# hzxie/GaussianCity

Measured on AMD Instinct MI355X. Metric: rendered frames/sec (fwd) @ 5000000 Gaussians, 1920x1080, higher is better.
Workload: dtype f32; 1 GPU; C3: s_city 5000000 Gaussians, 1920x1080, SH degree 3, forward, 24-pose orbit; exp=gcr-fp32-v2 (bit-exact vs oracle), tile_sort=lists beyond 1024 entries sorted lazily, as far as the blend walks (default), cull=stateless: every frame reads means, scales, rotations (default)

## Files before the change

### gaussiancity_amd/_native.py

```python
import ctypes as C
import subprocess

from . import _loader

GRAD_REC_FLOATS = 16

STAGE_NAMES = ("preprocess", "scan", "emit", "sort", "ranges", "blend_fwd", "blend_bwd",
               "preprocess_bwd")


class Options(C.Structure):
    _fields_ = [(n, C.c_int32) for n in (
        "lazy_sort", "sort_in_blend", "bwd_piece", "deterministic_backward", "split_preprocess",
        "force_radix", "force_global_cursor", "bwd_wave_units")]

    def __init__(self, **kw):
        super().__init__(*([-1] * 8))
        for k, v in kw.items():
            if k not in dict(self._fields_):
                raise TypeError("unknown rasterizer option %r" % k)
            setattr(self, k, int(v))


class Camera(C.Structure):
# ... 25 lines not shown
    ]


class Grads(C.Structure):
    _fields_ = [(n, C.c_void_p) for n in (
        "dL_dmeans2D", "dL_dconic", "dL_dopacity", "dL_dcolors", "dL_dmeans3D", "dL_dcov3D",
        "dL_dsh", "dL_dscales", "dL_drotations")] + [
        ("stride_means3D", C.c_int32), ("stride_opacity", C.c_int32), ("stride_colors", C.c_int32),
        ("stride_scales", C.c_int32), ("stride_rotations", C.c_int32),
        ("packed", C.c_void_p), ("packed_floats", C.c_int64)]


class Layout(C.Structure):
    _fields_ = [
        ("geom_rec", C.c_size_t), ("geom_cov3D", C.c_size_t), ("geom_clamped", C.c_size_t),
        ("geom_tiles_touched", C.c_size_t), ("geom_block_sums", C.c_size_t),
        ("geom_vis_list", C.c_size_t), ("geom_vis_count", C.c_size_t),
        ("geom_num_rendered", C.c_size_t), ("geom_block_tiles", C.c_size_t), ("geom_total", C.c_size_t),
        ("img_final_T", C.c_size_t), ("img_n_contrib", C.c_size_t), ("img_ranges", C.c_size_t),
        ("img_tile_cursor", C.c_size_t), ("img_tile_table", C.c_size_t), ("img_tile_lazy", C.c_size_t),
        ("img_total", C.c_size_t),
        ("bin_keys", C.c_size_t * 2), ("bin_vals", C.c_size_t * 2), ("bin_hist", C.c_size_t),
        ("bin_sorted", C.c_size_t), ("bin_work", C.c_size_t), ("bin_mask", C.c_size_t), ("bin_ckpt", C.c_size_t),
        ("bin_total", C.c_size_t), ("bin_lean_total", C.c_size_t), ("bin_staged", C.c_size_t),
        ("geom_vis_rec", C.c_size_t),
    ]


class FrameInfo(C.Structure):
    _fields_ = [("num_rendered", C.c_int64), ("max_tile_instances", C.c_int64)]


ABI_VERSION = 9
TICKET_WORDS = 8
RESIZE_FN = C.CFUNCTYPE(C.c_void_p, C.c_void_p, C.c_size_t)

_vp, _sz, _i32, _i64, _u32, _int = C.c_void_p, C.c_size_t, C.c_int32, C.c_int64, C.c_uint32, C.c_int
_cam, _gs, _info, _opts = C.POINTER(Camera), C.POINTER(Gaussians), C.POINTER(FrameInfo), C.POINTER(Options)
_SIGNATURES = {
    "gcr_abi_version": (_int, []),
    "gcr_last_error": (C.c_char_p, []),
    "gcr_geometry_bytes": (_sz, [_i32]),
    "gcr_image_bytes": (_sz, [_i32, _i32]),
    "gcr_binning_bytes": (_sz, [_i64, _i32, _i32]),
    "gcr_binning_bytes_lean": (_sz, [_i64, _i32, _i32]),
    "gcr_get_layout": (_int, [_i32, _i32, _i32, _i64, C.POINTER(Layout)]),
    "gcr_forward": (_int, [_cam, _gs, _vp, _sz, _vp, _sz, _i64, _i64, _vp, _sz, _vp, _vp, _info, _vp]),
    "gcr_forward_preprocess": (_int, [_cam, _gs, _vp, _sz, _vp, _sz, _vp, _info, _vp]),
    "gcr_forward_render": (_int, [_cam, _gs, _vp, _sz, _vp, _sz, _vp, _sz, _info, _vp, _vp]),
    "gcr_backward": (_int, [_cam, _gs, _vp, _vp, _sz, _vp, _sz, _vp, _sz, _i64, _vp, C.POINTER(Grads), _vp]),
    "gcr_build_cull_cache": (_int, [_gs, C.c_float, _vp, _vp]),
    "gcr_cull_cache_bytes": (_sz, [_i32]),
    "gcr_mark_visible": (_int, [_i32, _vp, _vp, _vp, _vp, _vp]),
    "gcr_rasterize_forward": (_i64, [RESIZE_FN, _vp, RESIZE_FN, _vp, RESIZE_FN, _vp, _cam, _gs, _vp, _vp, _vp]),
    "gcr_set_option": (_int, [C.c_char_p, _int]),
    "gcr_get_option": (_int, [C.c_char_p]),
    "gcr_get_stage_ms": (_int, [C.POINTER(C.c_float), _int]),
    "gcr_grad_record_floats": (_int, []),
    "gcr_grad_record_floats_opt": (_int, [_opts]),
    "gcr_forward_async": (_int, [_cam, _gs, _vp, _sz, _vp, _sz, _i64, _i64, _vp, _sz, _vp, _vp, _vp, _u32, _vp]),
    "gcr_ticket_poll": (_int, [_vp, _u32, _i64, _info]),
    "gcr_ticket_wait": (_int, [_vp, _u32, _i64, _vp, _info]),
    "gcr_host_words_alloc": (_vp, [_sz]),
    "gcr_host_words_free": (None, [_vp]),
    "gcr_rescue_count": (C.c_long, []),
    "gcr_rescue_dropped_count": (C.c_long, []),
# ... 34 lines not shown
```

### gaussiancity_amd/csrc/gcr_api.hip

```cpp
#include <atomic>
#include <chrono>
#include <condition_variable>
#include <cstdio>
#include <cstring>
#include <deque>
#include <map>
#include <mutex>
#include <string>
#include <thread>

#include <pthread.h>

#include "gcr_internal.h"
#define GC_ERR_HIP GCR_ERR_DEVICE
#include "gc_host.h"

namespace {

std::atomic<int> g_timing{0};
std::atomic<int> g_force_radix{0};
std::atomic<int> g_force_global_cursor{0};
std::atomic<int> g_lazy_sort{1};
std::atomic<int> g_sort_in_blend{0};
std::atomic<int> g_split_preprocess{0};
// ... 274 lines not shown

template <class A>
void set_gaussian_args(A& a, const gcr_gaussians* g) {
  a.P = g->P;
  a.means3D = g->means3D; a.scales = g->scales; a.rotations = g->rotations;
  a.s_mean = stride_or(g->stride_means3D, 3);
  a.s_scale = stride_or(g->stride_scales, 3);
  a.s_rot = stride_or(g->stride_rotations, 4);
}
template <class A>
void set_camera_args(A& a, const gcr_camera* cam, const gcr_gaussians* g) {
  set_gaussian_args(a, g);
  a.D = cam->sh_degree; a.M = g->M; a.W = cam->img_w; a.H = cam->img_h;
  a.tanfovx = cam->tanfovx; a.tanfovy = cam->tanfovy;
  a.focal_y = cam->img_h / (2.0f * cam->tanfovy);
  a.focal_x = cam->img_w / (2.0f * cam->tanfovx);
  a.scale_modifier = cam->scale_modifier;
  a.shs = g->shs;
  a.view = cam->view_matrix; a.proj = cam->proj_matrix; a.campos = cam->campos;
  fill_cam(a.cam, cam);
}

GcrBlendArgs blend_args(const FrameSetup& f, const gcr_camera* cam, const uint32_t* list) {
  GcrBlendArgs b;
  memset(&b, 0, sizeof(b));
  b.ranges = f.ranges;
  b.list = list;
  b.rec = f.rec;
  b.W = cam->img_w; b.H = cam->img_h; b.gx = f.gx; b.gy = f.gy;
  b.bg = cam->bg;
  b.flip_x = cam->flip_x != 0; b.flip_y = cam->flip_y != 0;
  b.win_x = cam->win_x; b.win_y = cam->win_y; b.win_w = cam->win_w; b.win_h = cam->win_h;
  b.out_u8 = cam->out_u8 != 0 && cam->backward != 1;
  fill_cam(b.cam, cam);
  b.final_T = f.final_T;
  b.n_contrib = f.n_contrib;
  return b;
}

}

extern "C" {

#ifdef GCR_EXPERIMENTS
void gcr_debug_set_clock_buffer(void* dev_ptr) { g_clock_buf.store((unsigned long long*)dev_ptr); }
#endif

int gcr_abi_version(void) { return GCR_ABI_VERSION; }
int gcr_grad_record_floats(void) { return g_deterministic.load() ? GCR_GRAD_REC_FLOATS_DET : GCR_GRAD_REC_FLOATS; }
int gcr_grad_record_floats_opt(const gcr_options* options) {
  return resolve_options(options).deterministic ? GCR_GRAD_REC_FLOATS_DET : GCR_GRAD_REC_FLOATS;
}
const char* gcr_last_error(void) { return g_err.c_str(); }

size_t gcr_geometry_bytes(int32_t P) { return compute_layout(P, 16, 16, 0).geom_total; }
size_t gcr_image_bytes(int32_t W, int32_t H) { return compute_layout(0, W, H, 0).img_total; }
size_t gcr_binning_bytes(int64_t R, int32_t W, int32_t H) { return compute_layout(0, W, H, R).bin_total; }
size_t gcr_binning_bytes_lean(int64_t R, int32_t W, int32_t H) { return compute_layout(0, W, H, R).bin_lean_total; }
int gcr_get_layout(int32_t P, int32_t W, int32_t H, int64_t R, gcr_layout* out) {
  if (!out) return fail(GCR_ERR_INVALID_ARGUMENT, "null layout");
  *out = compute_layout(P, W, H, R);
  return 0;
}

int gcr_set_option(const char* name, int value) {
  const OptionRow* o = find_option(name);
// ... 323 lines not shown
  std::condition_variable idle_cv_;

  static void publish(unsigned long long* w, int idx, unsigned int seq) {
    std::atomic_thread_fence(std::memory_order_seq_cst);
    ((volatile unsigned long long*)w)[idx] = (unsigned long long)seq;
    std::atomic_thread_fence(std::memory_order_seq_cst);
  }

  void rescue(AsyncFrame& f) {
    volatile unsigned long long* w = f.words;
    publish(f.words, 7, f.seq);
    if ((unsigned int)w[4] == f.seq) {
      publish(f.words, 5, f.seq);
      publish(f.words, 2, f.seq);
      dropped_.fetch_add(1);
      return;
    }
    const unsigned long long R = w[0] & 0xffffffffull;
    bool ok = false;
    void* stale = nullptr;
    do {
      if (check_num_rendered(R)) break;
      if (hipSetDevice(f.device) != hipSuccess) break;
      const int d = f.device & 63;
      if (!streams_[d]) {
        int lo = 0, hi = 0;
        if (hipDeviceGetStreamPriorityRange(&lo, &hi) != hipSuccess) lo = hi = 0;
        if (hipStreamCreateWithPriority(&streams_[d], hipStreamNonBlocking, hi) != hipSuccess &&
            hipStreamCreateWithFlags(&streams_[d], hipStreamNonBlocking) != hipSuccess)
          break;
      }
      hipStream_t s = streams_[d];
      gcr_camera cam = f.cam;
      cam.backward = 0;
      cam.options = f.has_opt ? &f.opt : nullptr;
      if (cam.host_camera) {
        cam.view_matrix = f.camvals;
        cam.proj_matrix = f.camvals + 16;
        cam.campos = f.camvals + 32;
        cam.bg = f.camvals + 35;
      }
      const FrameSetup fs = frame_setup(resolve_options(cam.options), f.g.P, &cam, 0, f.geom, f.img, nullptr);
      gcr_frame_info info;
      info.num_rendered = (int64_t)R;
      unsigned long long longest = 0;
      if (hipMemcpyAsync(&longest, fs.frame + 1, 8, hipMemcpyDeviceToHost, s) != hipSuccess) break;
      if (hipStreamSynchronize(s) != hipSuccess) break;
      info.max_tile_instances = (int64_t)longest;
      const size_t bytes = gcr_binning_bytes_lean((int64_t)R, cam.img_w, cam.img_h);
      if (scratch_bytes_[d] < bytes) {
        stale = scratch_[d];
        scratch_[d] = nullptr;
        scratch_bytes_[d] = 0;
        if (hipMalloc(&scratch_[d], bytes + bytes / 2) != hipSuccess) {
          scratch_[d] = nullptr;
          break;
        }
        scratch_bytes_[d] = bytes + bytes / 2;
      }
      if (gcr_forward_render(&cam, &f.g, f.geom, f.geom_bytes, scratch_[d], scratch_bytes_[d], f.img, f.img_bytes, &info,
                             f.out_color, s) < 0)
        break;
      if (hipStreamSynchronize(s) != hipSuccess) break;
      ok = true;
    } while (false);
    if (!ok) publish(f.words, 5, f.seq);
    publish(f.words, 6, f.seq);
// ... 428 lines not shown
```

### gaussiancity_amd/csrc/gcr_binning.hip

```cpp
#include <stdlib.h>
#include "gcr_device.h"
#include "gcr_internal.h"
#include "gcr_sort.h"

namespace {

constexpr int SORT_THREADS = 256;
constexpr int SORT_ITEMS = 16;
constexpr int SORT_TILE = SORT_THREADS * SORT_ITEMS;
constexpr int RADIX_BITS = 8;
constexpr int RADIX = 1 << RADIX_BITS;

__global__ __launch_bounds__(256) void k_emit(int P, const uint32_t* __restrict__ tiles_touched,
                                              const uint32_t* __restrict__ block_offsets,
                                              const float4* __restrict__ rec, int gx,
                                              uint64_t* __restrict__ keys,
                                              uint32_t* __restrict__ vals) {
  __shared__ uint32_t lds4[4];
  const int idx = blockIdx.x * 256 + threadIdx.x;
  const uint32_t t = idx < P ? tiles_touched[idx] : 0u;
  uint32_t total;
  uint32_t off = gcr_block_excl_scan_256(t, lds4, &total);
  if (t == 0) return;
  off += block_offsets[blockIdx.x];
// ... 54 lines not shown
      lo = mid;
    else
      hi = mid;
  }
  return (uint32_t)lo * (uint32_t)chunk + (f - pre[lo]);
}
GCR_DEV uint4 tt_survivor(const uint32_t* pre, int nblocks, const uint4* __restrict__ vis_rec, int chunk, uint32_t f) {
  return vis_rec[tt_position(pre, nblocks, chunk, f)];
}

template <bool SCATTER, int TT_THREADS>
__global__ __launch_bounds__(TT_THREADS) void k_tile_table(int T, int gx, int G, int nblocks_k1, int chunk,
                                                           const uint4* __restrict__ vis_rec,
                                                           const uint32_t* __restrict__ vis_count,
                                                           uint32_t* __restrict__ table,
                                                           const uint32_t* __restrict__ tile_total,
                                                           const uint32_t* __restrict__ tile_local,
                                                           const uint32_t* __restrict__ blk_total,
                                                           uint32_t* __restrict__ ranges,
                                                           uint64_t* __restrict__ pairs,
                                                           unsigned long long* __restrict__ frame,
                                                           unsigned long long cap_instances,
                                                           unsigned long long cap_list,
                                                           unsigned long long* __restrict__ host_word,
                                                           unsigned int seq,
                                                           const unsigned long long* __restrict__ block_tiles,
                                                           const uint4* __restrict__ banded, int banded_capacity) {
  extern __shared__ __attribute__((aligned(16))) unsigned char gcr_smem[];
  uint32_t* cnt = reinterpret_cast<uint32_t*>(gcr_smem);
  __shared__ uint32_t pre[GCR_K1_MAX_BLOCKS + 1];
  __shared__ uint32_t blk_base[TT_MAX_TBLOCKS];
  __shared__ uint32_t wtot[TT_THREADS / 64];
  const int tid = threadIdx.x, lane = tid & 63, w = tid >> 6;
  uint32_t* __restrict__ row = table + (size_t)blockIdx.x * T;
  TtPrefix<TT_THREADS> blocks;
  blocks.load(vis_count, nblocks_k1, tid);
  if (!SCATTER) {
    if (blockIdx.x == 0) {
      unsigned long long part = 0ull, pf = 0ull;
      for (int b = tid; b < nblocks_k1; b += TT_THREADS) {
        const unsigned long long v = block_tiles[b];
        part += v & ~GCR_PREFILTER_FLAG;
        pf |= v & GCR_PREFILTER_FLAG;
      }
#pragma unroll
      for (int o = 32; o > 0; o >>= 1) part += __shfl_xor(part, o, 64);
      __shared__ unsigned long long wpart[TT_THREADS / 64];
      if (lane == 0) wpart[w] = part;
      const int prefilter_violation = __syncthreads_or(pf != 0ull ? 1 : 0);
      if (tid == 0) {
        unsigned long long total = 0ull;
#pragma unroll
        for (int k = 0; k < TT_THREADS / 64; k++) total += wpart[k];
        if (prefilter_violation) total = GCR_PREFILTER_MARK;
        frame[0] = total;
        frame[1] = 0ull;
        frame[2] = 0ull;
        frame[GCR_FRAME_PIECE] = 0ull;
        frame[GCR_FRAME_BANDED] = banded != nullptr ? 1ull : 0ull;
        if (host_word != nullptr)
          gcr_store_to_host(host_word, ((unsigned long long)seq << 32) | (total > 0xffffffffull ? 0xffffffffull : total));
      }
    }
    for (int t = tid; t < T; t += TT_THREADS) cnt[t] = 0u;
  } else {
    const bool go = frame[0] <= cap_instances && frame[1] <= cap_list;
    if (blockIdx.x == 0 && tid == 0) {
// ... 500 lines not shown
  k_emit<<<(P + 255) / 256, 256, 0, s>>>(P, tiles_touched, block_offsets, rec, gx, keys, vals);
  return hipGetLastError();
}

bool gcr_band_sort_possible(int T) { return T >= GCR_BANDS; }

int gcr_tile_table_groups(int T, int nblocks_k1, int* G_out) {
  const size_t lds = (size_t)T * sizeof(uint32_t);
  if (lds > 148 * 1024 || (T + 63) / 64 > TT_MAX_TBLOCKS) return 0;
  int ng = 128;
#ifdef GCR_EXPERIMENTS
  if (const char* e = getenv("GCR_TT_GROUPS")) ng = atoi(e);
#endif
  if (ng > nblocks_k1) ng = nblocks_k1;
  if (ng < 1) ng = 1;
  int G = (nblocks_k1 + ng - 1) / ng;
  *G_out = G;
  return (nblocks_k1 + G - 1) / G;
}

static hipError_t tile_table_attr() {
  static hipError_t done = [] {
    const void* fns[4] = {(const void*)k_tile_table<false, 512>, (const void*)k_tile_table<true, 512>,
                          (const void*)k_tile_table<false, 1024>, (const void*)k_tile_table<true, 1024>};
    for (const void* f : fns) {
      const hipError_t e = hipFuncSetAttribute(f, hipFuncAttributeMaxDynamicSharedMemorySize, 148 * 1024);
      if (e != hipSuccess) return e;
    }
    return hipSuccess;
  }();
  return done;
}
static inline bool tile_table_wide(int) { return true; }

hipError_t gcr_launch_tile_count(int T, int gx, int NG, int G, int nblocks_k1, int chunk, const uint4* vis_rec,
                                 const uint32_t* vis_count, uint32_t* table,
                                 uint32_t* tile_total, uint32_t* tile_local, uint32_t* blk_total,
                                 unsigned long long* frame, const unsigned long long* block_tiles,
                                 unsigned long long* host_R, unsigned int seq, uint4* banded, int banded_capacity,
                                 hipStream_t s) {
  hipError_t e = tile_table_attr();
  if (e != hipSuccess) return e;
  if (banded != nullptr) {
    const uint32_t band_mul = (uint32_t)((((uint64_t)GCR_BANDS << 32) + (uint64_t)T - 1) / (uint64_t)T);
    k_band<false><<<BAND_CUTS, BAND_THREADS, 0, s>>>(gx, band_mul, nblocks_k1, chunk, vis_rec, vis_count, table, nullptr,
                                                      banded_capacity);
    k_band<true><<<BAND_CUTS, BAND_THREADS, 0, s>>>(gx, band_mul, nblocks_k1, chunk, vis_rec, vis_count, table, banded,
                                                     banded_capacity);
  }
  if (tile_table_wide(T))
    k_tile_table<false, 1024><<<NG, 1024, (size_t)T * sizeof(uint32_t), s>>>(
        T, gx, G, nblocks_k1, chunk, vis_rec, vis_count, table, nullptr, nullptr, nullptr, nullptr, nullptr,
        frame, 0ull, 0ull, host_R, seq, block_tiles, banded, banded_capacity);
  else
    k_tile_table<false, 512><<<NG, 512, (size_t)T * sizeof(uint32_t), s>>>(
        T, gx, G, nblocks_k1, chunk, vis_rec, vis_count, table, nullptr, nullptr, nullptr, nullptr, nullptr,
        frame, 0ull, 0ull, host_R, seq, block_tiles, banded, banded_capacity);
  k_table_colscan<<<(T + 63) / 64, 1024, 0, s>>>(table, NG, T, tile_total, tile_local, blk_total, frame);
  return hipGetLastError();
}

hipError_t gcr_launch_tile_scatter(int T, int gx, int NG, int G, int nblocks_k1, int chunk, const uint4* vis_rec,
                                   const uint32_t* vis_count, uint32_t* table,
                                   const uint32_t* tile_total, const uint32_t* tile_local,
                                   const uint32_t* blk_total, uint32_t* ranges, uint64_t* pairs,
                                   unsigned long long* frame, unsigned long long cap_instances,
                                   unsigned long long cap_list, unsigned long long* host_longest,
                                   const uint4* banded, int banded_capacity, hipStream_t s) {
  hipError_t e = tile_table_attr();
  if (e != hipSuccess) return e;
  if (tile_table_wide(T))
    k_tile_table<true, 1024><<<NG, 1024, (size_t)T * sizeof(uint32_t), s>>>(
        T, gx, G, nblocks_k1, chunk, vis_rec, vis_count, table, tile_total, tile_local, blk_total, ranges, pairs,
        frame, cap_instances, cap_list, host_longest, 0u, nullptr, banded, banded_capacity);
  else
    k_tile_table<true, 512><<<NG, 512, (size_t)T * sizeof(uint32_t), s>>>(
        T, gx, G, nblocks_k1, chunk, vis_rec, vis_count, table, tile_total, tile_local, blk_total, ranges, pairs,
        frame, cap_instances, cap_list, host_longest, 0u, nullptr, banded, banded_capacity);
  return hipGetLastError();
}

__global__ __launch_bounds__(256) void k_restore_cursors(const uint32_t* __restrict__ ranges,
                                                         uint32_t* __restrict__ cursor, int T) {
  const int t = blockIdx.x * 256 + threadIdx.x;
  if (t < T) cursor[(size_t)t * GCR_CURSOR_STRIDE] = ranges[2 * t];
}

hipError_t gcr_launch_scatter_instances(int nblocks, int chunk, const uint32_t* vis_list,
                                        const uint32_t* vis_count, const float4* rec, int gx,
                                        uint32_t* tile_cursor, uint64_t* pairs, const uint32_t* ranges, int T,
                                        const unsigned long long* frame, hipStream_t s) {
  if (nblocks <= 0) return hipSuccess;
  if (frame == nullptr)
    k_restore_cursors<<<(T + 255) / 256, 256, 0, s>>>(ranges, tile_cursor, T);
  k_scatter_instances<<<nblocks, 256, 0, s>>>(chunk, vis_list, vis_count, rec, gx, tile_cursor, pairs, frame);
  return hipGetLastError();
}

__global__ __launch_bounds__(256) void k_fill_tiles_touched(int chunk, const uint32_t* __restrict__ vis_list,
                                                            const uint32_t* __restrict__ vis_count,
                                                            const float4* __restrict__ rec,
                                                            uint32_t* __restrict__ tiles_touched) {
  const uint32_t nvis = vis_count[blockIdx.x];
  const uint32_t* __restrict__ my_list = vis_list + (size_t)blockIdx.x * chunk;
  for (uint32_t it = threadIdx.x; it < nvis; it += 256) {
    const uint32_t idx = my_list[it];
    const float4 q2 = rec[(size_t)idx * GCR_REC_QUADS + 2];
    const uint32_t rx = __float_as_uint(q2.z), ry = __float_as_uint(q2.w);
    tiles_touched[idx] = ((rx >> 16) - (rx & 0xffffu)) * ((ry >> 16) - (ry & 0xffffu));
  }
// ... 86 lines not shown
```

### gaussiancity_amd/csrc/gcr_blend.hip

```cpp
#include "gcr_cull.h"
#include "gcr_device.h"
#include "gcr_internal.h"
#include "gcr_sort.h"

namespace {

constexpr int CHUNK = 256;
constexpr uint32_t ENTRY_BYTES = 48;
constexpr int K6_SENT_SLOT = 223;
constexpr int K6_LIST_STRIDE = 232;
static_assert(GCR_PIECE_MAX <= K6_SENT_SLOT, "a K6 chunk must leave slot 255 to the sentinel");
constexpr uint32_t NO_ENTRY = 0xFFFFFFFFu;

struct __attribute__((aligned(16))) StagedEntry {
  float4 a, b, c;
};
static_assert(sizeof(StagedEntry) == ENTRY_BYTES, "StagedEntry must be 48 bytes");

GCR_DEV float gcr_alpha_skip_bound(float opacity) {
  if (!(opacity > 0.0f)) return __builtin_inff();
  return gcr_max(-87.0f, -__builtin_logf(255.0f * opacity) - 1.0e-3f);
}

GCR_DEV float blend_exp(float x) { return gcr_expf_noguard(x); }
// ... 107 lines not shown
  uint32_t ns = __hip_atomic_load(w, __ATOMIC_RELAXED, __HIP_MEMORY_SCOPE_AGENT);
  uint64_t l = (uint64_t)__hip_atomic_load(w + 2, __ATOMIC_RELAXED, __HIP_MEMORY_SCOPE_AGENT) |
               ((uint64_t)__hip_atomic_load(w + 3, __ATOMIC_RELAXED, __HIP_MEMORY_SCOPE_AGENT) << 32);
  gcr_lazy_extend<GCR_LAZY_CAP_K6>(s, keys, n, ns, l, out, tid);
  if (tid == 0) {
    __hip_atomic_store(w, ns, __ATOMIC_RELAXED, __HIP_MEMORY_SCOPE_AGENT);
    __hip_atomic_store(w + 2, (uint32_t)l, __ATOMIC_RELAXED, __HIP_MEMORY_SCOPE_AGENT);
    __hip_atomic_store(w + 3, (uint32_t)(l >> 32), __ATOMIC_RELAXED, __HIP_MEMORY_SCOPE_AGENT);
  }
  __syncthreads();
  return ns;
}

__device__ __noinline__ void k6_frame_gate(unsigned long long* words, unsigned int seq, unsigned int max_polls) {
  gcr_store_to_host(words + 3, (unsigned long long)seq);
  for (unsigned int i = 0; i < max_polls; i++) {
    const unsigned long long v = __hip_atomic_load(words + 2, __ATOMIC_RELAXED, __HIP_MEMORY_SCOPE_SYSTEM);
    if ((unsigned int)v == seq) return;
    __builtin_amdgcn_s_sleep(127);
    __builtin_amdgcn_s_sleep(127);
  }
  gcr_store_to_host(words + 4, (unsigned long long)seq);
  asm volatile("s_waitcnt vmcnt(0)" ::: "memory");
  const unsigned long long st = __hip_atomic_load(words + 7, __ATOMIC_RELAXED, __HIP_MEMORY_SCOPE_SYSTEM);
  if ((unsigned int)st != seq) return;
  for (unsigned long long i = 0; i < 16ull * max_polls; i++) {
    const unsigned long long v = __hip_atomic_load(words + 2, __ATOMIC_RELAXED, __HIP_MEMORY_SCOPE_SYSTEM);
    if ((unsigned int)v == seq) return;
    __builtin_amdgcn_s_sleep(127);
    __builtin_amdgcn_s_sleep(127);
  }
}

template <bool SORT, bool STATE>
__global__ __launch_bounds__(256) __attribute__((amdgpu_waves_per_eu(8, 8))) void k_blend_fwd(const GcrBlendArgs a) {
  __shared__ StagedEntry sE[K6_SENT_SLOT + 1];
  __shared__ uint32_t sMask[CHUNK];
  __shared__ __attribute__((aligned(16))) uint8_t sList[4][8][K6_LIST_STRIDE];

  if (a.frame != nullptr && a.frame[2] == 0ull) {
    if (a.gate_words != nullptr && blockIdx.x == 0 && threadIdx.x == 0) k6_frame_gate(a.gate_words, a.gate_seq, a.gate_polls);
    return;
  }
  const int tile = blockIdx.x;
  const int tx = tile % a.gx, ty = tile / a.gx;
  const int tid = threadIdx.x;
  const float tile_x0 = (float)(tx * GCR_TILE_X), tile_y0 = (float)(ty * GCR_TILE_Y);
  const uint32_t r0 = a.ranges[2 * tile], r1 = a.ranges[2 * tile + 1];
  if (!gcr_tile_in_window(a, tx, ty)) {
    if (STATE && a.work != nullptr) {
      const uint32_t P0 = (uint32_t)a.piece, sb = r0 / P0 + (uint32_t)tile, ns = r1 / P0 + 1u - r0 / P0;
      for (uint32_t k = tid; k < ns; k += 256u) a.work[sb + k] = make_uint4(GCR_NO_TILE, 0u, 0u, 0u);
      if (tile == 0 && tid == 0) {
        a.frame_out[GCR_FRAME_PIECE] = P0;
        a.frame_out[GCR_FRAME_CKPT_OFF] = a.ckpt_off;
        a.frame_out[GCR_FRAME_WORK_OFF] = a.work_off;
        a.frame_out[GCR_FRAME_MASK_OFF] = a.mask_off;
        a.frame_out[GCR_FRAME_STAGED_OFF] = a.staged_off;
        a.frame_out[GCR_FRAME_CARVE] = a.carve_bytes;
      }
    }
    return;
  }
  const int total = (int)(r1 - r0);
  const char* const sEb = reinterpret_cast<const char*>(sE);
#ifdef GCR_EXPERIMENTS
  if (a.clock_buf != nullptr && tid == 0) {
// ... 52 lines not shown
      __syncthreads();
    } else {
      for (int i = tid; i < total; i += 256) {
        const uint64_t mine = seg[i];
        uint32_t rank = 0;
        for (int j = 0; j < total; j++) rank += seg[j] < mine ? 1u : 0u;
        out[rank] = (uint32_t)mine;
      }
      __syncthreads();
    }
  }

#define GCR_BLEND_STEP(QA, QB, QC, OFF)                                                      \
  {                                                                                          \
    const float dx = QA.x - pixx, dy = QA.y - pixy;                                          \
    const float power = __builtin_fmaf(QA.w * dx, dy, __builtin_fmaf(QB.x * dy, dy, (QA.z * dx) * dx)); \
    const bool in_range = !(power > 0.0f) && !(power < QC.y);                                \
    if (GCR_K6_WAVE_SKIP(in_range) && GCR_K6_STEP_ON) {                     \
        \
      const float araw = __builtin_fminf(0.99f, QB.y * blend_exp(power));          \
      const bool valid = in_range && !(araw < 1.0f / 255.0f);                                \
      const float a_eff = valid ? araw : 0.0f;                                               \
      const float test_T = Tw * (1 - a_eff);                                                 \
      const bool keep = !(test_T < 0.0001f);                                                 \
      const float wgt = keep ? a_eff : 0.0f;                                                 \
      C0 = __builtin_fmaf(QB.z * wgt, Tw, C0);                                               \
      C1 = __builtin_fmaf(QB.w * wgt, Tw, C1);                                               \
      C2 = __builtin_fmaf(QC.x * wgt, Tw, C2);                                               \
      if (STATE) {     \
        D0 = __builtin_fmaf(QB.z * wgt, Tw, D0);                                             \
        D1 = __builtin_fmaf(QB.w * wgt, Tw, D1);                                             \
        D2 = __builtin_fmaf(QC.x * wgt, Tw, D2);                                             \
      }                                                                                      \
      last_off = (keep && valid) ? (OFF) : last_off;                                         \
      Tw = keep ? test_T : -__builtin_fabsf(Tw);                                             \
    }                                                                                        \
  }
#define GCR_BLEND_LOAD(QA, QB, QC, OFF)                            \
  QA = *reinterpret_cast<const float4*>(sEb + (OFF));             \
  QB = *reinterpret_cast<const float4*>(sEb + (OFF) + 16);         \
  QC = *reinterpret_cast<const float2*>(sEb + (OFF) + 32);

  int base = 0;
  bool finished = false;
  while (base < total && !finished && GCR_K6_LOOP_ON) {
  if (!SORT) {
    const uint32_t need = (uint32_t)(base + min(cs, total - base));
    while (lz_sorted < need) {
      const uint32_t ns = k6_lazy_extend(reinterpret_cast<uint64_t*>(sE), a.pairs + r0, (uint32_t)total,
                                         a.list_out + r0, a.lazy + tile);
      lz_sorted = (uint32_t)__builtin_amdgcn_readfirstlane((int)ns);
    }
  }
  int tid_op = threadIdx.x;
  asm volatile("" : "+v"(tid_op));
  const LaneGeom6 g = lane_geom6(tid_op, tx, ty);
  const int lane = g.lane;
  const float pixx = (float)g.pxi, pixy = (float)g.pyi;
  const int w_u = __builtin_amdgcn_readfirstlane(g.w);
  const int mask_sh = (w_u >> 1) * 16 + (w_u & 1) * 4;
  uint8_t* const lw = &sList[w_u][0][0];
  for (; base < total; base += cs) {
    if (__syncthreads_count(!(Tw > 0.0f)) == 256) {
      finished = true;
      break;
    }
    if (!SORT && lz_sorted < (uint32_t)(base + min(cs, total - base))) break;
// ... 72 lines not shown
        }
      }
    }
    const int maxcnt = __builtin_amdgcn_readfirstlane(
        max(max(max(cnt[0], cnt[1]), max(cnt[2], cnt[3])), max(max(cnt[4], cnt[5]), max(cnt[6], cnt[7]))));
    __builtin_amdgcn_wave_barrier();
#ifdef GCR_EXPERIMENTS
    if (a.clock_buf != nullptr && tid == 0 && base == 0) {
      a.clock_buf[(size_t)tile * 16 + 5] = __builtin_readcyclecounter();
      a.clock_buf[(size_t)tile * 16 + 7] = (unsigned long long)maxcnt;
    }
#endif
    const uint8_t* lp = &sList[w_u][g.sub][0];
    float4 qa0, qb0, qa1, qb1;
    float2 qc0, qc1;
    uint32_t e0 = (uint32_t)lp[0] * ENTRY_BYTES, e1 = (uint32_t)lp[1] * ENTRY_BYTES;
    uint32_t last_off = NO_ENTRY;
    GCR_BLEND_LOAD(qa0, qb0, qc0, e0)
    for (int i = 0; i < maxcnt; i += 2, lp += 2) {
      GCR_BLEND_LOAD(qa1, qb1, qc1, e1)
      const uint32_t cur0 = e0;
      e0 = (uint32_t)lp[2] * ENTRY_BYTES;
      GCR_BLEND_STEP(qa0, qb0, qc0, cur0)
      if (i + 1 >= maxcnt) break;
      GCR_BLEND_LOAD(qa0, qb0, qc0, e0)
      const uint32_t cur1 = e1;
      e1 = (uint32_t)lp[3] * ENTRY_BYTES;
      GCR_BLEND_STEP(qa1, qb1, qc1, cur1)
      if (__ballot(Tw > 0.0f) == 0ull) break;
    }
#ifdef GCR_EXPERIMENTS
    if (a.clock_buf != nullptr && tid == 0 && base == 0) a.clock_buf[(size_t)tile * 16 + 6] = __builtin_readcyclecounter();
#endif
    if (last_off != NO_ENTRY) last_contributor = (uint32_t)base + slot_of_offset(last_off) + 1u;
  }
  }
#undef GCR_BLEND_STEP
#undef GCR_BLEND_LOAD
  int tid_end = threadIdx.x;
  asm volatile("" : "+v"(tid_end));
  const LaneGeom6 g = lane_geom6(tid_end, tx, ty);
  if (g.pxi < a.W && g.pyi < a.H && (!STATE || a.out_color != nullptr)) {
    const float Tout = __builtin_fabsf(Tw);
    const size_t pix_id = (size_t)a.W * g.pyi + g.pxi;
    const bool nt_out = !STATE && a.nt_out != 0;
    if (nt_out) {
      __builtin_nontemporal_store(Tout, a.final_T + pix_id);
      __builtin_nontemporal_store(last_contributor, a.n_contrib + pix_id);
    } else {
      a.final_T[pix_id] = Tout;
      a.n_contrib[pix_id] = last_contributor;
    }
    size_t oplane;
    int px_op = g.pxi, py_op = g.pyi;
    asm volatile("" : "+v"(px_op), "+v"(py_op));
    const long long out_id = gcr_out_index(a, px_op, py_op, &oplane);
    if (out_id >= 0) {
      const float c0 = C0 + Tout * GCR_CAM(a, bg, a.bg, 0);
      const float c1 = C1 + Tout * GCR_CAM(a, bg, a.bg, 1);
      const float c2 = C2 + Tout * GCR_CAM(a, bg, a.bg, 2);
      if (!STATE && a.out_u8) {
        uint8_t* o = reinterpret_cast<uint8_t*>(a.out_color) + 3 * (size_t)out_id;
        o[0] = gcr_video_byte(c0);
        o[1] = gcr_video_byte(c1);
        o[2] = gcr_video_byte(c2);
      } else if (nt_out) {
        __builtin_nontemporal_store(c0, a.out_color + out_id);
        __builtin_nontemporal_store(c1, a.out_color + oplane + out_id);
        __builtin_nontemporal_store(c2, a.out_color + 2 * oplane + out_id);
      } else {
        a.out_color[out_id] = c0;
        a.out_color[oplane + out_id] = c1;
        a.out_color[2 * oplane + out_id] = c2;
      }
    }
  }
#ifdef GCR_EXPERIMENTS
  if (a.clock_buf != nullptr && tid == 0) a.clock_buf[(size_t)tile * 16 + 2] = __builtin_readcyclecounter();
#endif
  if (STATE && a.work != nullptr) {
    if (entered >= 2u)
      a.ckpt[(size_t)(sbase + entered - 1u) * 256u + lane6_to_k7_thread((uint32_t)tid)] =
          make_float4(__builtin_fabsf(Tw), D0, D1, D2);
    const uint32_t nslots = r1 / piece_P + 1u - r0 / piece_P;
    for (uint32_t k = tid; k < nslots; k += 256u)
      a.work[sbase + k] = k < entered ? make_uint4((uint32_t)tile, r0, (uint32_t)total, k) : make_uint4(GCR_NO_TILE, 0u, 0u, 0u);
  }
  if (STATE && a.work != nullptr && tile == 0 && tid == 0) {
    a.frame_out[GCR_FRAME_PIECE] = piece_P;
// ... 513 lines not shown
        GCR_BWD_STEP(qa0, qb0, qc0)
        if (i + 1 >= maxcnt) break;
        GCR_BWD_LOAD(qa0, qb0, qc0, e0)
        e1 = (uint32_t)lp[3] * ENTRY_BYTES;
        GCR_BWD_STEP(qa1, qb1, qc1)
      }
    }
    __syncthreads();
    {
      const int comp = tid & 15;
      const int rec_idx = comp < 3 ? comp : (comp == 8 ? 3 : comp + 1);
      if (comp < 9 && GCR_FLUSH_ON) {
        for (int i = tid >> 4; i < n; i += 16) {
          const float v = (float)sAcc[i * 9 + comp];
          if (v != 0.0f) atomicAdd(&a.grad_rec[(size_t)sId[i] * GCR_GRAD_REC_FLOATS + rec_idx], v);
        }
      }
    }
  }
}

#undef GCR_BWD_STEP
#undef GCR_BWD_LOAD

}

template <bool SORT>
static void launch_blend_fwd_state(const GcrBlendArgs& a, int T, hipStream_t s) {
  size_t pad = 0;
#ifdef GCR_EXPERIMENTS
  if (const char* e = getenv("GCR_K6_LDS_PAD")) pad = (size_t)atoll(e);
#endif
  if (a.work != nullptr)
    k_blend_fwd<SORT, true><<<T, 256, pad, s>>>(a);
  else
    k_blend_fwd<SORT, false><<<T, 256, pad, s>>>(a);
}

hipError_t gcr_launch_blend_fwd(const GcrBlendArgs& a, bool sort_in_kernel, hipStream_t s) {
  const int T = a.gx * a.gy;
  if (T <= 0) return hipSuccess;
  if (sort_in_kernel)
    launch_blend_fwd_state<true>(a, T, s);
  else
    launch_blend_fwd_state<false>(a, T, s);
  return hipGetLastError();
}

hipError_t gcr_launch_blend_bwd(const GcrBlendArgs& a, bool wave_units, hipStream_t s) {
  const int T = a.gx * a.gy;
  if (T <= 0) return hipSuccess;
  unsigned long long items = gcr_piece_slots(a.R, (unsigned long long)T, (unsigned long long)a.piece);
  if (wave_units || a.deterministic) {
    unsigned long long units = (4ull * items + 31ull) & ~31ull;
#ifdef GCR_EXPERIMENTS
    if (const char* env = getenv("GCR_K7_BLOCKS")) units = (unsigned long long)atoll(env);
#endif
    const unsigned int grid = (unsigned int)(units > 0x3fffffe0ull ? 0x3fffffe0ull : units) + (unsigned int)a.fill.blocks;
    k_blend_bwd<<<grid, 64, 0, s>>>(a);
  } else {
    GcrBlendArgs b = a;
    b.fill.blocks = (a.fill.blocks + 3) / 4;
    const unsigned int grid = (unsigned int)(items > 0x3fffffffull ? 0x3fffffffull : items) + (unsigned int)b.fill.blocks;
    k_blend_bwd_item<<<grid, 256, 0, s>>>(b);
  }
  return hipGetLastError();
}
```

### gaussiancity_amd/csrc/gcr_internal.h

```cpp
#pragma once
#include <hip/hip_runtime.h>
#include <stdint.h>

#include "../../include/gcr.h"

#define GCR_REC_QUADS 4
#define GCR_COV3D_FLOATS 8

#define GCR_CURSOR_STRIDE 32

struct GcrCamVals {
  int by_value;
  float view[16], proj[16], campos[3], bg[3];
};
#define GCR_CAM(A, FIELD, PTR, i) ((A).cam.by_value ? (A).cam.FIELD[i] : (PTR)[i])

struct GcrPreprocessArgs {
  int P, D, M, W, H, gx, gy;
  float tanfovx, tanfovy, focal_x, focal_y, scale_modifier;
  const float *means3D, *scales, *rotations, *opacities, *shs, *cov3D_precomp, *colors_precomp;
  const float *view, *proj, *campos;
  int32_t* radii;
  float4* rec;
  float* cov3D;
  uint32_t* tile_count;
  uint32_t* vis_list;
  uint32_t* vis_count;
  uint4* vis_rec;
  uint32_t* cand_list;
  uint32_t* cand_count;
  unsigned long long* block_tiles;
  int nblocks, chunk;
  int s_mean, s_opac, s_col, s_scale, s_rot;
  int prefiltered;
  const float4* cull_cache;
  const float4* cull_shape;
  int nt_stream;
// ... 83 lines not shown
}
#define GCR_FRAME_PIECE 3
#define GCR_FRAME_CKPT_OFF 4
#define GCR_FRAME_WORK_OFF 5
#define GCR_FRAME_MASK_OFF 7
#define GCR_FRAME_CARVE 6
#define GCR_FRAME_STAGED_OFF 8
#define GCR_BAND_SORT_MIN_DEFAULT 6000000
#define GCR_FRAME_BANDED 9
static inline __host__ __device__ bool gcr_frame_has_state(const unsigned long long* frame, unsigned long long binning_bytes) {
  return frame[GCR_FRAME_PIECE] != 0ull && frame[GCR_FRAME_CARVE] <= binning_bytes;
}

struct GcrBlendArgs {
  const uint32_t* ranges;
  const uint32_t* list;
  const uint64_t* pairs;
  uint32_t* list_out;
  const float4* rec;
  int W, H, gx, gy;
  const float* bg;
  float* final_T;
  uint32_t* n_contrib;
  float* out_color;
  const unsigned long long* frame;
  const float* dL_dpix;
  float* grad_rec;
  GcrFillArgs fill;
  int deterministic;
  int win_x, win_y, win_w, win_h;
  int flip_x, flip_y;
  int out_u8;
  int nt_out;
  GcrCamVals cam;
  int debug_flags;
  int piece;
  float4* ckpt;
  uint4* work;
  uint16_t* mask_out;
  unsigned long long mask_off;
  float4* staged_out;
  unsigned long long staged_off;
  unsigned long long* frame_out;
  unsigned long long ckpt_off, work_off;
  unsigned long long carve_bytes;
  unsigned long long* gate_words;
  unsigned int gate_seq, gate_polls;
  unsigned long long binning_bytes;
  const char* binning_base;
  const unsigned long long* frame_in;
  uint4* lazy;
  unsigned long long R;
#ifdef GCR_EXPERIMENTS
  unsigned long long* clock_buf;
#endif
};

hipError_t gcr_launch_mark_visible(int P, const float* means3D, const float* view, uint8_t* present,
                                   hipStream_t s);
hipError_t gcr_launch_preprocess(const GcrPreprocessArgs& a, bool split, hipStream_t s);
hipError_t gcr_launch_build_cull_cache(const GcrPreprocessArgs& a, float4* outA, float4* outB, hipStream_t s);
static inline size_t gcr_cull_cache_offset_b(int P) { return (((size_t)P * 16) + 127) & ~(size_t)127; }
hipError_t gcr_launch_zero_grad_records(int nblocks, int chunk, const uint32_t* vis_list, const uint32_t* vis_count,
                                        float4* grad_rec, int rec_quads, hipStream_t s);
hipError_t gcr_launch_fill(const GcrFillArgs& f, hipStream_t s);
hipError_t gcr_launch_scan_block_sums(uint32_t* block_sums, int n, unsigned long long* total,
// ... 58 lines not shown
```

### gaussiancity_amd/ext.py

```python
import collections
import ctypes as C
import os
import threading
import weakref

import torch

from . import _native as N
from . import cull_cache as _cull

NUM_CHANNELS = 3

_CAPACITY_HINT_MAX = 64
_capacity_hint = collections.OrderedDict()
_hint_lock = threading.Lock()


poison_outputs = False


_tls = threading.local()


def set_backward_hint(flag):
# ... 158 lines not shown
        return None, None
    if t.dtype != torch.float32:
        raise RuntimeError("%s must be float32 (got %s)" % (name, t.dtype))
    if t.device != device:
        raise RuntimeError("%s must live on %s (got %s)" % (name, device, t.device))
    if not t.is_contiguous():
        t = t.contiguous()
    return t, t.data_ptr()


def _camera(device, bg, view, proj, campos, tan_fovx, tan_fovy, H, W, scale_modifier, degree,
            prefiltered, debug, for_backward=False, flip_x=False, flip_y=False, window=None, out_u8=False):
    cams = ((bg, "bg", 3), (view, "viewmatrix", 16), (proj, "projmatrix", 16), (campos, "campos", 3))
    on_host = all(isinstance(t, torch.Tensor) and t.device.type == "cpu" and t.numel() != 0 for t, _, _ in cams)
    keep = []
    ptrs = []
    for t, name, n in cams:
        if on_host:
            if t.dtype != torch.float32:
                raise RuntimeError("%s must be float32 (got %s)" % (name, t.dtype))
            tt = t.contiguous()
            p = tt.data_ptr()
        else:
            tt, p = _dev_f32(t, name, device)
        if tt is None or tt.numel() != n:
            raise RuntimeError("%s must have %d elements" % (name, n))
        keep.append(tt)
        ptrs.append(p)
    cam = N.Camera(int(H), int(W), float(tan_fovx), float(tan_fovy), float(scale_modifier),
                   int(degree), int(bool(prefiltered)), int(bool(debug)), *ptrs)
    cam.host_camera = int(on_host)
    cam.flip_x = int(bool(flip_x))
    cam.flip_y = int(bool(flip_y))
    cam.backward = int(bool(for_backward))
    cam.out_u8 = int(bool(out_u8))
    opt = _current_options()
    if opt is not None:
        cam.options = C.pointer(opt)
        keep.append(opt)
    if window is not None:
        cam.win_x, cam.win_y, cam.win_w, cam.win_h = (int(v) for v in window)
    return cam, keep


def _gaussians(device, P, means3D, opacity, sh, colors, scales, rotations, cov3D_precomp):
    keep = []
    ptr = {}
    for t, name in ((means3D, "means3D"), (opacity, "opacity"), (sh, "sh"), (colors, "colors"),
                    (scales, "scales"), (rotations, "rotations"),
                    (cov3D_precomp, "cov3D_precomp")):
        tt, p = _dev_f32(t, name, device)
        keep.append(tt)
        ptr[name] = p
    M = 0
    if sh is not None and sh.numel() != 0:
        if sh.dim() != 3 or sh.size(0) != P or sh.size(2) != 3:
            raise RuntimeError("sh must have dimensions (num_points, M, 3)")
        M = int(sh.size(1))
    for t, name, last in ((opacity, "opacity", None), (colors, "colors", 3), (scales, "scales", 3),
                          (rotations, "rotations", 4), (cov3D_precomp, "cov3D_precomp", 6)):
        if t is not None and t.numel() != 0 and t.numel() != P * (last or 1):
            raise RuntimeError("%s has %d elements, expected %d" % (name, t.numel(), P * (last or 1)))
    g = N.Gaussians(int(P), M, ptr["means3D"], ptr["opacity"], ptr["sh"], ptr["colors"],
                    ptr["scales"], ptr["rotations"], ptr["cov3D_precomp"])
    return g, keep


# ... 143 lines not shown
    N.check(L.gcr_forward_render(C.byref(cam), C.byref(g), geom.data_ptr(), geom.numel(), binning.data_ptr(),
                                 binning.numel(), img.data_ptr(), img.numel(), C.byref(info), None, _stream(device)),
            "gcr_forward_render (state only)")
    return R, binning


def _num_points(t, name, cols):
    if t.dim() != 2 or t.size(1) != cols:
        raise RuntimeError("%s must have dimensions (num_points, %d)" % (name, cols))
    if not t.is_cuda:
        raise RuntimeError("%s must be a GPU tensor: this rasterizer has no CPU path" % name)
    return int(t.size(0))


def _empty_frame(device, H, W, mode):
    color = torch.zeros((NUM_CHANNELS, H, W), dtype=torch.float32, device=device)
    radii = torch.zeros((0,), dtype=torch.int32, device=device)
    if mode == _IMAGE:
        return color, radii
    e = torch.empty((0,), dtype=torch.uint8, device=device)
    R = FrameTicket(None, None, None, 0, 0, None, None, False, R=0) if mode == _TICKET else 0
    return R, color, radii, e, e.clone(), e.clone()


def _rasterize(mode, for_backward, background, means3D, colors, opacity, scales, rotations, scale_modifier, cov3D_precomp,
               viewmatrix, projmatrix, tan_fovx, tan_fovy, image_height, image_width, sh, degree, campos, prefiltered,
               debug):
    P = _num_points(means3D, "means3D", 3)
    L = N.lib()
    device = means3D.device
    H, W = int(image_height), int(image_width)
    if P == 0:
        return _empty_frame(device, H, W, mode)
    with _on_device(device):
        if _cull.enabled() and not for_backward:
            cam, keep_c = _camera(device, background, viewmatrix, projmatrix, campos, tan_fovx,
                                  tan_fovy, H, W, scale_modifier, degree, prefiltered, debug, for_backward)
            g, keep_g = _gaussians(device, P, means3D, opacity, sh, colors, scales, rotations,
                                   cov3D_precomp)
            keep = (keep_c, keep_g, _cull.attach(g, scale_modifier, (means3D, scales, rotations, cov3D_precomp, opacity),
                                                 device, _stream(device)))
        else:
            cam, g, keep = _records(device, P, H, W, background, means3D, colors, opacity, scales, rotations, scale_modifier,
                                    cov3D_precomp, viewmatrix, projmatrix, tan_fovx, tan_fovy, sh, degree, campos,
                                    bool(prefiltered), bool(debug), bool(for_backward), _current_options())
        out = _forward(L, device, cam, g, P, H, W, mode)
        del keep
    return out


def rasterize_gaussians(background, means3D, colors, opacity, scales, rotations, scale_modifier,
                        cov3D_precomp, viewmatrix, projmatrix, tan_fovx, tan_fovy, image_height,
                        image_width, sh, degree, campos, prefiltered, debug, _for_backward=None, _ticket=False):
    if _for_backward is None:
        _for_backward = getattr(_tls, "backward", None)
        _for_backward = True if _for_backward is None else _for_backward
    return _rasterize(_TICKET if _ticket else _INT, _for_backward, background, means3D, colors, opacity, scales, rotations,
                      scale_modifier, cov3D_precomp, viewmatrix, projmatrix, tan_fovx, tan_fovy, image_height, image_width,
                      sh, degree, campos, prefiltered, debug)


def rasterize_gaussians_ticket(*args, _for_backward=False):
    return rasterize_gaussians(*args, _for_backward=_for_backward, _ticket=True)


_PREP_MAX = 64


class _Prepared:
    __slots__ = ("refs", "ptrs", "cam", "g")


def _prep_cache():
    c = getattr(_tls, "prep", None)
    if c is None:
        c = _tls.prep = collections.OrderedDict()
    return c

# ... 193 lines not shown
```

### include/gcr.h

```cpp
#ifndef GCR_H_INCLUDED
#define GCR_H_INCLUDED

#include <stddef.h>
#include <stdint.h>

#ifdef __cplusplus
extern "C" {
#endif

#define GCR_ABI_VERSION 9
#define GCR_BLOCK_X 16
#define GCR_BLOCK_Y 16
#define GCR_NUM_CHANNELS 3

typedef enum gcr_status {
  GCR_OK = 0,
  GCR_ERR_INVALID_ARGUMENT = -1,
  GCR_ERR_BUFFER_TOO_SMALL = -2,
  GCR_ERR_OVERFLOW = -3,
  GCR_ERR_DEVICE = -4,
  GCR_ERR_ALLOC = -5
} gcr_status;

typedef struct gcr_options {
  int32_t lazy_sort;
  int32_t sort_in_blend;
  int32_t bwd_piece;
  int32_t deterministic_backward;
  int32_t split_preprocess;
  int32_t force_radix;
  int32_t force_global_cursor;
  int32_t bwd_wave_units;
} gcr_options;
#define GCR_OPTIONS_DEFAULT {-1, -1, -1, -1, -1, -1, -1, -1}

typedef struct gcr_camera {
  int32_t img_h, img_w;
  float tanfovx, tanfovy;
  float scale_modifier;
  int32_t sh_degree;
  int32_t prefiltered;
  int32_t debug;
  const float *bg;
  const float *view_matrix;
  const float *proj_matrix;
  const float *campos;
  int32_t host_camera;
  int32_t flip_x, flip_y;
  int32_t win_x, win_y, win_w, win_h;
  int32_t backward;
  const gcr_options *options;
  int32_t out_u8;
} gcr_camera;

typedef struct gcr_gaussians {
  int32_t P;
  int32_t M;
  const float *means3D;
  const float *opacities;
  const float *shs;
  const float *colors_precomp;
  const float *scales;
  const float *rotations;
  const float *cov3D_precomp;
  int32_t stride_means3D, stride_opacities, stride_colors, stride_scales, stride_rotations;
  const void *cull_cache;
} gcr_gaussians;

size_t gcr_cull_cache_bytes(int32_t P);
int gcr_build_cull_cache(const gcr_gaussians *g, float scale_modifier, void *cull_cache_out, void *hip_stream);

typedef struct gcr_grads {
  float *dL_dmeans2D;
  float *dL_dconic;
  float *dL_dopacity;
  float *dL_dcolors;
  float *dL_dmeans3D;
  float *dL_dcov3D;
  float *dL_dsh;
  float *dL_dscales;
  float *dL_drotations;
  int32_t stride_means3D, stride_opacity, stride_colors, stride_scales, stride_rotations;
  float *packed;
  int64_t packed_floats;
} gcr_grads;

// ... 101 lines not shown
```

Measured before the change: 5928 frames/s.

## Skip per-pixel final_T/n_contrib writes in image-only forward and remap tile-table rows per XCD

Adds an image-only forward mode that Python selects when only the image is requested without backward. In that mode the blend kernel is instantiated without the last-contributor tracking and the final_T/n_contrib stores, which cuts per-pixel global writes and a little register work. Separately, the tile-table kernel now maps block indices to rows in contiguous per-XCD chunks, so neighbouring rows tend to land on the same XCD for cache locality. The image-only path applies only to the non-sorting blend variant, and the row remap changes table ordering, which the column scan must tolerate.

Measured after the change: 6143 frames/s (median of 6 runs). +3.6%, better.

```diff
diff --git a/gaussiancity_amd/_native.py b/gaussiancity_amd/_native.py
--- a/gaussiancity_amd/_native.py
+++ b/gaussiancity_amd/_native.py
@@ -81,6 +81,7 @@
 
 
 ABI_VERSION = 9
+BACKWARD_IMAGE_ONLY = 2
 TICKET_WORDS = 8
 RESIZE_FN = C.CFUNCTYPE(C.c_void_p, C.c_void_p, C.c_size_t)
 
diff --git a/gaussiancity_amd/csrc/gcr_api.hip b/gaussiancity_amd/csrc/gcr_api.hip
--- a/gaussiancity_amd/csrc/gcr_api.hip
+++ b/gaussiancity_amd/csrc/gcr_api.hip
@@ -330,6 +330,7 @@
   b.flip_x = cam->flip_x != 0; b.flip_y = cam->flip_y != 0;
   b.win_x = cam->win_x; b.win_y = cam->win_y; b.win_w = cam->win_w; b.win_h = cam->win_h;
   b.out_u8 = cam->out_u8 != 0 && cam->backward != 1;
+  b.image_only = cam->backward == GCR_BACKWARD_IMAGE_ONLY;
   fill_cam(b.cam, cam);
   b.final_T = f.final_T;
   b.n_contrib = f.n_contrib;
@@ -719,7 +720,7 @@
       }
       hipStream_t s = streams_[d];
       gcr_camera cam = f.cam;
-      cam.backward = 0;
+      if (cam.backward == 1) cam.backward = 0;
       cam.options = f.has_opt ? &f.opt : nullptr;
       if (cam.host_camera) {
         cam.view_matrix = f.camvals;
diff --git a/gaussiancity_amd/csrc/gcr_binning.hip b/gaussiancity_amd/csrc/gcr_binning.hip
--- a/gaussiancity_amd/csrc/gcr_binning.hip
+++ b/gaussiancity_amd/csrc/gcr_binning.hip
@@ -110,7 +110,12 @@
   __shared__ uint32_t blk_base[TT_MAX_TBLOCKS];
   __shared__ uint32_t wtot[TT_THREADS / 64];
   const int tid = threadIdx.x, lane = tid & 63, w = tid >> 6;
-  uint32_t* __restrict__ row = table + (size_t)blockIdx.x * T;
+#ifdef GCR_EXPERIMENTS
+  const uint32_t my_row = G < 0 ? blockIdx.x : gcr_tt_row(blockIdx.x, gridDim.x);
+#else
+  const uint32_t my_row = gcr_tt_row(blockIdx.x, gridDim.x);
+#endif
+  uint32_t* __restrict__ row = table + (size_t)my_row * T;
   TtPrefix<TT_THREADS> blocks;
   blocks.load(vis_count, nblocks_k1, tid);
   if (!SCATTER) {
@@ -677,6 +682,13 @@
   return done;
 }
 static inline bool tile_table_wide(int) { return true; }
+static inline int tile_table_G(int G) {
+#ifdef GCR_EXPERIMENTS
+  static const bool numeric = getenv("GCR_TT_ROWS_NUMERIC") != nullptr && atoi(getenv("GCR_TT_ROWS_NUMERIC")) != 0;
+  if (numeric) return -1;
+#endif
+  return G;
+}
 
 hipError_t gcr_launch_tile_count(int T, int gx, int NG, int G, int nblocks_k1, int chunk, const uint4* vis_rec,
                                  const uint32_t* vis_count, uint32_t* table,
@@ -695,11 +707,11 @@
   }
   if (tile_table_wide(T))
     k_tile_table<false, 1024><<<NG, 1024, (size_t)T * sizeof(uint32_t), s>>>(
-        T, gx, G, nblocks_k1, chunk, vis_rec, vis_count, table, nullptr, nullptr, nullptr, nullptr, nullptr,
+        T, gx, tile_table_G(G), nblocks_k1, chunk, vis_rec, vis_count, table, nullptr, nullptr, nullptr, nullptr, nullptr,
         frame, 0ull, 0ull, host_R, seq, block_tiles, banded, banded_capacity);
   else
     k_tile_table<false, 512><<<NG, 512, (size_t)T * sizeof(uint32_t), s>>>(
-        T, gx, G, nblocks_k1, chunk, vis_rec, vis_count, table, nullptr, nullptr, nullptr, nullptr, nullptr,
+        T, gx, tile_table_G(G), nblocks_k1, chunk, vis_rec, vis_count, table, nullptr, nullptr, nullptr, nullptr, nullptr,
         frame, 0ull, 0ull, host_R, seq, block_tiles, banded, banded_capacity);
   k_table_colscan<<<(T + 63) / 64, 1024, 0, s>>>(table, NG, T, tile_total, tile_local, blk_total, frame);
   return hipGetLastError();
@@ -716,11 +728,11 @@
   if (e != hipSuccess) return e;
   if (tile_table_wide(T))
     k_tile_table<true, 1024><<<NG, 1024, (size_t)T * sizeof(uint32_t), s>>>(
-        T, gx, G, nblocks_k1, chunk, vis_rec, vis_count, table, tile_total, tile_local, blk_total, ranges, pairs,
+        T, gx, tile_table_G(G), nblocks_k1, chunk, vis_rec, vis_count, table, tile_total, tile_local, blk_total, ranges, pairs,
         frame, cap_instances, cap_list, host_longest, 0u, nullptr, banded, banded_capacity);
   else
     k_tile_table<true, 512><<<NG, 512, (size_t)T * sizeof(uint32_t), s>>>(
-        T, gx, G, nblocks_k1, chunk, vis_rec, vis_count, table, tile_total, tile_local, blk_total, ranges, pairs,
+        T, gx, tile_table_G(G), nblocks_k1, chunk, vis_rec, vis_count, table, tile_total, tile_local, blk_total, ranges, pairs,
         frame, cap_instances, cap_list, host_longest, 0u, nullptr, banded, banded_capacity);
   return hipGetLastError();
 }
diff --git a/gaussiancity_amd/csrc/gcr_blend.hip b/gaussiancity_amd/csrc/gcr_blend.hip
--- a/gaussiancity_amd/csrc/gcr_blend.hip
+++ b/gaussiancity_amd/csrc/gcr_blend.hip
@@ -163,7 +163,7 @@
   }
 }
 
-template <bool SORT, bool STATE>
+template <bool SORT, bool STATE, bool PIXSTATE>
 __global__ __launch_bounds__(256) __attribute__((amdgpu_waves_per_eu(8, 8))) void k_blend_fwd(const GcrBlendArgs a) {
   __shared__ StagedEntry sE[K6_SENT_SLOT + 1];
   __shared__ uint32_t sMask[CHUNK];
@@ -282,7 +282,7 @@
         D1 = __builtin_fmaf(QB.w * wgt, Tw, D1);                                             \
         D2 = __builtin_fmaf(QC.x * wgt, Tw, D2);                                             \
       }                                                                                      \
-      last_off = (keep && valid) ? (OFF) : last_off;                                         \
+      if (PIXSTATE) last_off = (keep && valid) ? (OFF) : last_off;                           \
       Tw = keep ? test_T : -__builtin_fabsf(Tw);                                             \
     }                                                                                        \
   }
@@ -421,7 +421,7 @@
 #ifdef GCR_EXPERIMENTS
     if (a.clock_buf != nullptr && tid == 0 && base == 0) a.clock_buf[(size_t)tile * 16 + 6] = __builtin_readcyclecounter();
 #endif
-    if (last_off != NO_ENTRY) last_contributor = (uint32_t)base + slot_of_offset(last_off) + 1u;
+    if (PIXSTATE && last_off != NO_ENTRY) last_contributor = (uint32_t)base + slot_of_offset(last_off) + 1u;
   }
   }
 #undef GCR_BLEND_STEP
@@ -429,21 +429,23 @@
   int tid_end = threadIdx.x;
   asm volatile("" : "+v"(tid_end));
   const LaneGeom6 g = lane_geom6(tid_end, tx, ty);
-  if (g.pxi < a.W && g.pyi < a.H && (!STATE || a.out_color != nullptr)) {
+  static_assert(PIXSTATE || !STATE, "the backward reads final_T / n_contrib");
+  if (g.pxi < a.W && g.pyi < a.H) {
     const float Tout = __builtin_fabsf(Tw);
     const size_t pix_id = (size_t)a.W * g.pyi + g.pxi;
     const bool nt_out = !STATE && a.nt_out != 0;
-    if (nt_out) {
+    if (!PIXSTATE) {
+    } else if (nt_out) {
       __builtin_nontemporal_store(Tout, a.final_T + pix_id);
       __builtin_nontemporal_store(last_contributor, a.n_contrib + pix_id);
     } else {
       a.final_T[pix_id] = Tout;
       a.n_contrib[pix_id] = last_contributor;
     }
-    size_t oplane;
+    size_t oplane = 0;
     int px_op = g.pxi, py_op = g.pyi;
     asm volatile("" : "+v"(px_op), "+v"(py_op));
-    const long long out_id = gcr_out_index(a, px_op, py_op, &oplane);
+    const long long out_id = (!STATE || a.out_color != nullptr) ? gcr_out_index(a, px_op, py_op, &oplane) : -1;
     if (out_id >= 0) {
       const float c0 = C0 + Tout * GCR_CAM(a, bg, a.bg, 0);
       const float c1 = C1 + Tout * GCR_CAM(a, bg, a.bg, 1);
@@ -1023,9 +1025,11 @@
   if (const char* e = getenv("GCR_K6_LDS_PAD")) pad = (size_t)atoll(e);
 #endif
   if (a.work != nullptr)
-    k_blend_fwd<SORT, true><<<T, 256, pad, s>>>(a);
+    k_blend_fwd<SORT, true, true><<<T, 256, pad, s>>>(a);
+  else if (!SORT && a.image_only)
+    k_blend_fwd<false, false, false><<<T, 256, pad, s>>>(a);
   else
-    k_blend_fwd<SORT, false><<<T, 256, pad, s>>>(a);
+    k_blend_fwd<SORT, false, true><<<T, 256, pad, s>>>(a);
 }
 
 hipError_t gcr_launch_blend_fwd(const GcrBlendArgs& a, bool sort_in_kernel, hipStream_t s) {
diff --git a/gaussiancity_amd/csrc/gcr_internal.h b/gaussiancity_amd/csrc/gcr_internal.h
--- a/gaussiancity_amd/csrc/gcr_internal.h
+++ b/gaussiancity_amd/csrc/gcr_internal.h
@@ -3,6 +3,7 @@
 #include <stdint.h>
 
 #include "../../include/gcr.h"
+#include "gcr_tt_row.h"
 
 #define GCR_REC_QUADS 4
 #define GCR_COV3D_FLOATS 8
@@ -152,6 +153,7 @@
   int flip_x, flip_y;
   int out_u8;
   int nt_out;
+  int image_only;
   GcrCamVals cam;
   int debug_flags;
   int piece;
diff --git a/gaussiancity_amd/csrc/gcr_tt_row.h b/gaussiancity_amd/csrc/gcr_tt_row.h
--- /dev/null
+++ b/gaussiancity_amd/csrc/gcr_tt_row.h
@@ -0,0 +1,14 @@
+#pragma once
+
+#if defined(__HIPCC__)
+#define GCR_TT_ROW_FN __host__ __device__ inline __attribute__((always_inline))
+#else
+#define GCR_TT_ROW_FN static inline
+#endif
+
+#define GCR_XCDS 8
+
+GCR_TT_ROW_FN unsigned gcr_tt_row(unsigned b, unsigned NG) {
+  const unsigned c = b % GCR_XCDS, q = NG / GCR_XCDS, r = NG % GCR_XCDS;
+  return c * q + (c < r ? c : r) + b / GCR_XCDS;
+}
diff --git a/gaussiancity_amd/ext.py b/gaussiancity_amd/ext.py
--- a/gaussiancity_amd/ext.py
+++ b/gaussiancity_amd/ext.py
@@ -214,7 +214,7 @@
     cam.host_camera = int(on_host)
     cam.flip_x = int(bool(flip_x))
     cam.flip_y = int(bool(flip_y))
-    cam.backward = int(bool(for_backward))
+    cam.backward = N.BACKWARD_IMAGE_ONLY if for_backward == N.BACKWARD_IMAGE_ONLY else int(bool(for_backward))
     cam.out_u8 = int(bool(out_u8))
     opt = _current_options()
     if opt is not None:
@@ -424,10 +424,11 @@
     H, W = int(image_height), int(image_width)
     if P == 0:
         return _empty_frame(device, H, W, mode)
+    state = N.BACKWARD_IMAGE_ONLY if (mode == _IMAGE and not for_backward) else bool(for_backward)
     with _on_device(device):
         if _cull.enabled() and not for_backward:
             cam, keep_c = _camera(device, background, viewmatrix, projmatrix, campos, tan_fovx,
-                                  tan_fovy, H, W, scale_modifier, degree, prefiltered, debug, for_backward)
+                                  tan_fovy, H, W, scale_modifier, degree, prefiltered, debug, state)
             g, keep_g = _gaussians(device, P, means3D, opacity, sh, colors, scales, rotations,
                                    cov3D_precomp)
             keep = (keep_c, keep_g, _cull.attach(g, scale_modifier, (means3D, scales, rotations, cov3D_precomp, opacity),
@@ -435,7 +436,7 @@
         else:
             cam, g, keep = _records(device, P, H, W, background, means3D, colors, opacity, scales, rotations, scale_modifier,
                                     cov3D_precomp, viewmatrix, projmatrix, tan_fovx, tan_fovy, sh, degree, campos,
-                                    bool(prefiltered), bool(debug), bool(for_backward), _current_options())
+                                    bool(prefiltered), bool(debug), state, _current_options())
         out = _forward(L, device, cam, g, P, H, W, mode)
         del keep
     return out
diff --git a/include/gcr.h b/include/gcr.h
--- a/include/gcr.h
+++ b/include/gcr.h
@@ -52,6 +52,7 @@
   const gcr_options *options;
   int32_t out_u8;
 } gcr_camera;
+#define GCR_BACKWARD_IMAGE_ONLY 2
 
 typedef struct gcr_gaussians {
   int32_t P;
```
